# ucl-bug/helmnet

Hardware: AMD Instinct MI355X
Metric: solver iterations/sec (whole node), 256^2 domain batch=32 (higher is better)
Workload: dtype f32

## Files before the change

### helmnet_amd/_lib.py

```python
from __future__ import annotations

import ctypes
import os
from ctypes import POINTER, c_char_p, c_double, c_float, c_int, c_int64, c_size_t, c_void_p

import torch

_LIB_PATH = os.environ.get("HELMNET_HIP_LIB") or os.path.join(os.path.dirname(os.path.abspath(__file__)), "libhelmnet_hip.so")
_lib = None

HN_ACT = {"prelu": 0, "relu": 1, "leakyrelu": 2, "celu": 3, "tanh": 4, "gelu": 5, "tanhshrink": 6, "softplus": 7}
HN_PRECISION = {"fp32": 0, "bf16x3": 1, "fp16": 2, "bf16x2": 3, "valu": 4}
HN_OPTION = {"lanes": 0, "side_stream": 1, "deep": 3, "spectral_pfa": 4, "spectral_radix16": 5, "dc_valu": 6, "spectral_cols": 7, "train_fused": 10, "train_overlap": 11, "dc_pair": 12, "side_sync": 13, "state_kernel": 14, "hist_copy": 15, "inc_sigma_map": 16, "spectral_mixed": 17,
             "graph": 100, "train_lanes": 101, "spectral_plain": 102}
HN_COUNTER = {"graph_replays": 0, "eager_iterations": 1, "graphs_captured": 2, "stream_probes": 3, "side_candidate": 4, "train_fwd_events": 5, "flag_sync_iterations": 6, "spectral_route": 7}
ABI_VERSION = 7
HN_VJP = {"continue": 1, "defer": 2}

SYMBOLS = {
    "hn_abi_version": (c_int, []),
    "hn_create": (c_int, [POINTER(c_void_p), c_int]),
    "hn_destroy": (None, [c_void_p]),
    "hn_last_error": (c_char_p, [c_void_p]),
    "hn_set_unet_precision": (c_int, [c_void_p, c_int]),
    "hn_get_unet_precision": (c_int, [c_void_p]),
    "hn_set_option": (c_int, [c_void_p, c_int, c_int]),
    "hn_get_counter": (c_int64, [c_void_p, c_int]),
    "hn_check_async_errors": (c_int, [c_void_p]),
    "hn_weight_count": (c_size_t, [c_int, c_int, c_int]),
    "hn_load_weights": (c_int, [c_void_p, POINTER(c_float), c_size_t, c_int, c_int, c_int, c_int]),
    "hn_set_domain": (c_int, [c_void_p, c_int, c_int, c_float, c_float]),
    "hn_get_sigmas": (c_int, [c_void_p, c_void_p, c_void_p]),
    "hn_state_len": (c_int64, [c_void_p]),
    "hn_reserve": (c_int, [c_void_p, c_int]),
    "hn_laplacian": (c_int, [c_void_p, c_void_p, c_void_p, c_int, c_void_p]),
    "hn_residual": (c_int, [c_void_p, c_void_p, c_void_p, c_void_p, c_int, c_void_p, c_int, c_void_p]),
    "hn_residual_vjp": (c_int, [c_void_p, c_void_p, c_void_p, c_void_p, c_int, c_void_p]),
    "hn_rmse": (c_int, [c_void_p, c_void_p, c_void_p, c_int, c_void_p]),
    "hn_laplacian_f64": (c_int, [c_void_p, c_void_p, c_void_p, c_int, c_void_p]),
    "hn_residual_f64": (c_int, [c_void_p, c_void_p, c_void_p, c_void_p, c_int, c_void_p, c_void_p, c_int, c_void_p]),
    "hn_gmres_cycle": (c_int, [c_void_p, c_void_p, c_void_p, c_void_p, c_int, c_int, c_int, c_float, c_void_p, c_void_p, c_void_p, c_void_p, c_void_p]),
    "hn_gmres_refine_cycle": (c_int, [c_void_p, c_void_p, c_void_p, c_void_p, c_int, c_int, c_int, c_double, c_float, c_void_p, c_void_p, c_void_p, c_void_p,
                                      c_void_p, c_void_p]),
    "hn_fgmres_cycle": (c_int, [c_void_p, c_void_p, c_void_p, c_void_p, c_int, c_int, c_int, c_float, c_int, c_float, c_void_p, c_void_p, c_void_p, c_void_p,
                                c_void_p, c_void_p]),
    "hn_fgmres_refine_cycle": (c_int, [c_void_p, c_void_p, c_void_p, c_void_p, c_int, c_int, c_int, c_double, c_float, c_int, c_float, c_void_p, c_void_p,
# ... 71 lines not shown
```

### helmnet_amd/csrc/hn_api.hip

```cpp
#include <cmath>
#include <cstdlib>
#include <cstring>

#include <cstdio>
#include "hn_internal.h"

namespace hn {

static thread_local std::string g_err;

void set_global_error(const char* msg) { g_err = msg; }

int fail(hn_ctx* ctx, int code, const char* fmt, ...) {
    char buf[512];
    va_list ap;
    va_start(ap, fmt);
    vsnprintf(buf, sizeof(buf), fmt, ap);
    va_end(ap);
    if (ctx) ctx->err = buf;
    g_err = buf;
    return code;
}

ProfScope::ProfScope(hn_ctx* ctx, int id, hipStream_t st) : c(ctx), s(st) {
// ... 208 lines not shown
    if (!out) return fail(nullptr, HN_ERR_ARG, "hn_create: out is NULL");
    *out = nullptr;
    int count = 0;
    hipError_t e = hipGetDeviceCount(&count);
    if (e != hipSuccess || count == 0)
        return fail(nullptr, HN_ERR_HIP, "hn_create: no HIP device available (%s)", hipGetErrorString(e));
    if (device_id < 0 || device_id >= count) return fail(nullptr, HN_ERR_ARG, "hn_create: device %d of %d", device_id, count);
    hipDeviceProp_t prop;
    if ((e = hipGetDeviceProperties(&prop, device_id)) != hipSuccess)
        return fail(nullptr, HN_ERR_HIP, "hipGetDeviceProperties: %s", hipGetErrorString(e));
    if (std::strncmp(prop.gcnArchName, "gfx950", 6) != 0)
        return fail(nullptr, HN_ERR_UNSUPPORTED, "device %d is %s; this library is built for gfx950 only", device_id, prop.gcnArchName);
    int prev = -1;
    (void)hipGetDevice(&prev);
    if ((e = hipSetDevice(device_id)) != hipSuccess) return fail(nullptr, HN_ERR_HIP, "hipSetDevice: %s", hipGetErrorString(e));
    if (prev >= 0 && prev != device_id) (void)hipSetDevice(prev);
    hn_ctx* c = new (std::nothrow) hn_ctx();
    if (!c) return fail(nullptr, HN_ERR_NOMEM, "out of host memory");
    c->device = device_id;
    *out = c;
    auto bad_env = [&](const char* name, const char* v) {
        const std::string why = c->err;
        hn_destroy(c);
        *out = nullptr;
        return fail(nullptr, HN_ERR_ARG, "hn_create: environment variable %s=%s rejected (%s)", name, v, why.c_str());
    };
    if (const char* v = getenv("HN_UNET_IMPL")) {
        const int mode = std::strcmp(v, "fp32") == 0 ? HN_PREC_FP32 : std::strcmp(v, "bf16x3") == 0 ? HN_PREC_BF16X3 : std::strcmp(v, "fp16") == 0 ? HN_PREC_FP16
                       : std::strcmp(v, "bf16x2") == 0 ? HN_PREC_BF16X2 : std::strcmp(v, "valu") == 0 ? HN_PREC_FP32_VALU : -1;
        if (hn_set_unet_precision(c, mode) != HN_OK) return bad_env("HN_UNET_IMPL", v);
    }
    const struct { const char* env; int opt; } knobs[] = {{"HN_STREAMS", HN_OPT_LANES}, {"HN_SIDE_STREAM", HN_OPT_SIDE_STREAM},
                                                            {"HN_GRAPH", HN_EXP_GRAPH}, {"HN_DEEP", HN_OPT_DEEP},
                                                            {"HN_TRAIN_LANES", HN_EXP_TRAIN_LANES}, {"HN_TRAIN_FUSED", HN_OPT_TRAIN_FUSED}, {"HN_TRAIN_OVERLAP", HN_OPT_TRAIN_OVERLAP}, {"HN_DC_VALU", HN_OPT_DC_VALU}, {"HN_DC_PAIR", HN_OPT_DC_PAIR}, {"HN_SIDE_SYNC", HN_OPT_SIDE_SYNC}, {"HN_STATE_KERNEL", HN_OPT_STATE_KERNEL}, {"HN_HIST_COPY", HN_OPT_HIST_COPY}, {"HN_INC_SIGMA_MAP", HN_OPT_INC_SIGMA_MAP}, {"HN_SPECTRAL_MIXED", HN_OPT_SPECTRAL_MIXED}, {"HN_SPECTRAL_PLAIN", HN_EXP_SPECTRAL_PLAIN}};
    for (const char* name : {"ROCPROF_COUNTER_COLLECTION", "ROCPROF_COUNTERS", "ROCP_METRICS"})
        if (const char* v = getenv(name))
            if (v[0] != '\0' && std::strcmp(v, "0") != 0 && std::strcmp(v, "False") != 0 && std::strcmp(v, "false") != 0) c->opt_side_sync = 0;
    if (const char* v = getenv("HN_SIDE_PRIORITY")) { const int p = std::atoi(v); c->opt_side_priority = p < 0 || p > 3 ? 0 : p; }
    if (const char* v = getenv("HN_DEFER_JOIN")) c->opt_defer_join = std::atoi(v) != 0;
    for (const auto& k : knobs)
        if (const char* v = getenv(k.env)) {
            char* end = nullptr;
            const long n = std::strtol(v, &end, 10);
            if (end == v || *end != '\0') { c->err = "not an integer"; return bad_env(k.env, v); }
            if (hn_set_option(c, k.opt, (int)n) != HN_OK) return bad_env(k.env, v);
        }
    *out = c;
    return HN_OK;
}

int hn_set_unet_precision(hn_ctx* ctx, int precision) {
    if (!ctx) return HN_ERR_ARG;
    if (precision < HN_PREC_FP32 || precision > HN_PREC_FP32_VALU)
        return fail(ctx, HN_ERR_ARG, "hn_set_unet_precision: unknown mode %d", precision);
    if (precision != ctx->precision) clear_step_graphs(ctx);
    ctx->precision = precision;
    return HN_OK;
}

int hn_get_unet_precision(const hn_ctx* ctx) { return ctx ? ctx->precision : HN_ERR_ARG; }

int hn_set_option(hn_ctx* ctx, int option, int value) {
    if (!ctx) return HN_ERR_ARG;
    switch (option) {
        case HN_OPT_LANES:
            if (value < 1 || value > 8) return fail(ctx, HN_ERR_ARG, "HN_OPT_LANES must be in [1, 8] (got %d)", value);
            ctx->opt_lanes = value;
            break;
        case HN_OPT_SIDE_STREAM:
            if (value < 0 || value > 3) return fail(ctx, HN_ERR_ARG, "HN_OPT_SIDE_STREAM must be in [0, 3] (got %d)", value);
            ctx->opt_side_stream = value;
            break;
        case HN_EXP_GRAPH:
            if (value < 0 || value > 64 || (value > 1 && (value & 1)))
                return fail(ctx, HN_ERR_ARG, "HN_EXP_GRAPH must be 0, 1 or an even number of iterations per graph <= 64 (got %d)", value);
            ctx->opt_graph = value;
            break;
        case HN_OPT_DEEP:
            if (value < 0 || value > 2) return fail(ctx, HN_ERR_ARG, "HN_OPT_DEEP must be 0, 1 or 2 (got %d)", value);
            ctx->opt_deep = value;
            break;
        case HN_OPT_SPECTRAL_PFA:
            if (value < 0 || value > 1) return fail(ctx, HN_ERR_ARG, "HN_OPT_SPECTRAL_PFA must be 0 or 1 (got %d)", value);
            ctx->opt_pfa = value;
            break;
        case HN_OPT_SPECTRAL_MIXED:
            if (value < 0 || value > 1) return fail(ctx, HN_ERR_ARG, "HN_OPT_SPECTRAL_MIXED must be 0 or 1 (got %d)", value);
            ctx->opt_mixed = value;
            break;
        case HN_OPT_DC_VALU:
            if (value < 0 || value > 4) return fail(ctx, HN_ERR_ARG, "HN_OPT_DC_VALU must be 0 .. 4 (got %d)", value);
            ctx->opt_dc_valu = value;
            break;
        case HN_OPT_DC_PAIR:
            if (value < 0 || value > 1) return fail(ctx, HN_ERR_ARG, "HN_OPT_DC_PAIR must be 0 or 1 (got %d)", value);
            ctx->opt_dc_pair = value;
            break;
        case HN_OPT_STATE_KERNEL:
            if (value < 0 || value > 1) return fail(ctx, HN_ERR_ARG, "HN_OPT_STATE_KERNEL must be 0 or 1 (got %d)", value);
            ctx->opt_state_kernel = value;
            break;
        case HN_OPT_INC_SIGMA_MAP:
            if (value < 0 || value > 1) return fail(ctx, HN_ERR_ARG, "HN_OPT_INC_SIGMA_MAP must be 0 or 1 (got %d)", value);
            ctx->opt_inc_sigma_map = value;
            break;
        case HN_OPT_HIST_COPY:
            if (value < 0 || value > 1) return fail(ctx, HN_ERR_ARG, "HN_OPT_HIST_COPY must be 0 or 1 (got %d)", value);
            ctx->opt_hist_copy = value;
            break;
        case HN_OPT_SIDE_SYNC:
            if (value < 0 || value > 1) return fail(ctx, HN_ERR_ARG, "HN_OPT_SIDE_SYNC must be 0 or 1 (got %d)", value);
            ctx->opt_side_sync = value;
            break;
        case HN_OPT_SPECTRAL_RADIX16:
            if (value < 0 || value > 2) return fail(ctx, HN_ERR_ARG, "HN_OPT_SPECTRAL_RADIX16 must be 0, 1 or 2 (got %d)", value);
            ctx->opt_radix16 = value;
            break;
        case HN_OPT_SPECTRAL_COLS:
            if (value < 0 || value > 3) return fail(ctx, HN_ERR_ARG, "HN_OPT_SPECTRAL_COLS must be 0, 1, 2 or 3 (got %d)", value);
            ctx->opt_cols_t = value;
            break;
        case HN_EXP_SPECTRAL_PLAIN:
            if (value < 0 || value > 1) return fail(ctx, HN_ERR_ARG, "HN_EXP_SPECTRAL_PLAIN must be 0 or 1 (got %d)", value);
            ctx->opt_spec_plain = value;
            break;
        case HN_EXP_TRAIN_LANES:
            if (value < 1 || value > 2) return fail(ctx, HN_ERR_ARG, "HN_EXP_TRAIN_LANES must be 1 or 2 (got %d)", value);
            ctx->opt_train_lanes = value;
            break;
        case HN_OPT_TRAIN_FUSED:
            if (value < 0 || value > 63) return fail(ctx, HN_ERR_ARG, "HN_OPT_TRAIN_FUSED must be 0 .. 63 (got %d)", value);
            ctx->opt_train_fused = value;
            break;
// ... 730 lines not shown
```

### helmnet_amd/csrc/hn_internal.h

```cpp
#pragma once
#include <hip/hip_runtime.h>

#include <complex>
#include <cstdarg>
#include <cstdint>
#include <cstdio>
#include <string>
#include <vector>

#include "helmnet_hip.h"

namespace hn {

constexpr int kFeat = 8;
constexpr int kCounterStride = 32;
constexpr int kState = 2;
constexpr int kInCh = 6;
constexpr int kMaxDepth = 6;

struct Src {
    const float* p;
    long sb;
    long sc;
    float scale;
// ... 173 lines not shown
    hn::F64Unet* f64 = nullptr;
    hn::KrylovWs* kry = nullptr;
    hn::RefineWs* rfn = nullptr;
    hn::PrecondWs* pcw = nullptr;
    hn::DcLayer inc{}, sig[hn::kMaxDepth]{}, st[hn::kMaxDepth]{}, dec[hn::kMaxDepth + 1]{};
    hn::K8Layer down[hn::kMaxDepth]{}, up[hn::kMaxDepth]{};
    float* fragdev = nullptr;
    const float *f_dec0c = nullptr, *dec0c_b = nullptr;
    const float* v_dec0c = nullptr;
    bool deep_attr_set = false, pfa_attr_set = false, pfa_adj_attr_set = false;
    int precision = HN_PREC_FP32;
    int opt_lanes = 1;
    int opt_side_stream = 1;
    int opt_side_priority = 0;
    int opt_defer_join = 0;
    int opt_graph = 0;
    int opt_pfa = 1;
    int opt_mixed = 0;
    int opt_radix16 = 1;
    int opt_cols_t = 1;
    bool cols_t_attr_set = false, cols512_attr_set = false;
    int opt_spec_plain = 0;
    int opt_deep = 2;
    unsigned* dx_flags = nullptr;
    unsigned* dx_done = nullptr;
    bool deepx_attr_set = false;
    int opt_dc_valu = 4;
    int opt_dc_pair = 1;
    unsigned* pair_flags = nullptr;
    long pair_flags_cap = 0;
    unsigned pair_epoch = 0;
    unsigned* pair_done = nullptr;
    int opt_hist_copy = 0;
    int opt_state_kernel = 1;
    int opt_side_sync = 1;
    unsigned* sync_flags = nullptr;
    unsigned sync_epoch = 0;
    int* sync_err = nullptr;
    int* sync_err_dev = nullptr;
    hn_stream_verdict_rec* stream_tab = nullptr;
    hn_stream_verdict_rec* stream_tab_dev = nullptr;
    int stream_tab_cap = 0;
    float2* inc_sigma_map = nullptr;
    int inc_sigma_band = 0;
    float inc_w_sigma[144]{};
    int opt_inc_sigma_map = 1;
    const float* zero_page = nullptr;
    const float* outc_w = nullptr;
    const float* outc_b = nullptr;
    hn::SpecTables tab;
    int64_t state_len = 0;
    int64_t state_off[hn::kMaxDepth]{};
    int cap_batch = 0;
    float* buf_a[hn::kMaxDepth + 1]{};
    float* buf_o[hn::kMaxDepth]{};
    float* buf_y[hn::kMaxDepth + 1]{};
    float* st_tmp = nullptr;
    struct SideLane {
        hipStream_t stream = nullptr; hipEvent_t ev[hn::kMaxDepth]{}; hipEvent_t done = nullptr;
        bool pending = false;
    };
    SideLane side[8];
    struct SidePick {
        hipStream_t cand[4]{};
        struct Known { hipStream_t ref[3]{}; int nref = 0; int chosen = 0; };
        std::vector<Known> known;
// ... 262 lines not shown
```

### helmnet_amd/csrc/hn_mfma.hip

```cpp
#include <cstdlib>

#include "hn_internal.h"
#include <cstring>
#include <cstdint>

namespace hn {
namespace {

typedef float f32x4 __attribute__((ext_vector_type(4)));
typedef float f32x2 __attribute__((ext_vector_type(2)));

constexpr int cdiv_(int a, int b) { return (a + b - 1) / b; }
constexpr int cmax_(int a, int b) { return a > b ? a : b; }

__device__ __forceinline__ f32x4 mfma4(float a, float b, f32x4 c) {
    return __builtin_amdgcn_mfma_f32_16x16x4f32(a, b, c, 0, 0, 0);
}
__device__ __forceinline__ float div1000(float x) {
    const float r = 1e-3f;
    const float qv = x * r;
    const float e = fmaf(-qv, 1000.0f, x);
    return fmaf(e, r, qv);
}
template <int N>
__device__ __forceinline__ void interleave_mfma_dsread() {
#pragma unroll
    for (int i = 0; i < N; ++i) {
        __builtin_amdgcn_sched_group_barrier(0x008, 1, 0);
        __builtin_amdgcn_sched_group_barrier(0x100, 1, 0);
    }
}

template <int CA, int CB, int CC, int TW>
struct McCfg {
    static constexpr int TH = 16;
    static constexpr int CIN = CA + CB + CC;
    static constexpr int CK = 2;
    static constexpr int NG = cdiv_(CIN, CK);
    static constexpr int IR = TH + 4, PI = TW + 4;
// ... 1636 lines not shown
        for (int gi = 0; gi < C::GW2; ++gi) acc2[gi] = (f32x4){0.f, 0.f, 0.f, 0.f};
        mfma_pairs<C::GW2>(acc2, lds, boff2, MID, MPLANE, PM, F_A2 + 24 * 64, kFeat / 2, lane);
        mfma_pairs<C::GW2>(acc2, lds, boff2, MID + kFeat * MPLANE, MPLANE, PM, F_A2S, kState / 2, lane);
        store(a.dst[1], 2 * q, acc2);
    }
    {
        f32x4 acc2[C::GW2];
#pragma unroll
        for (int gi = 0; gi < C::GW2; ++gi) acc2[gi] = (f32x4){0.f, 0.f, 0.f, 0.f};
        mfma_pairs<C::GW2>(acc2, lds, boff2, MID + kFeat * MPLANE, MPLANE, PM, F_A2S + 6 * 64, kState / 2, lane, 6);
        if (q == 0) store(x.dst, 0, acc2);
    }
}

template <int WX>
struct DnCfg {
    static constexpr int WY = 4 / WX;
    static constexpr int TH = 16, TW = 16 * WX;
    static constexpr int R = TH / WY;
    static constexpr int NWIN = R + 2;
    static constexpr int IR = 2 * TH + 6;
    static constexpr int IC = 2 * TW + 6;
    static constexpr int PI = IC | 1;
    static constexpr int PLANE = IR * PI;
    static constexpr int PLANE_P = PLANE + 64;
    static constexpr int NT = 256;
    static constexpr int NL = cdiv_(IR * IC, NT);
};

template <int WX, bool ALL>
__global__ __launch_bounds__(256, 2) void k_down_mfma(Src in, Dst out, const float* __restrict__ afr ,
                                                       const float* __restrict__ bias, int Hin, int Win, SyncHook hook) {
    using C = DnCfg<WX>;
    sync_hook_begin(hook);
    __shared__ float lds[(ALL ? kFeat : 2) * C::PLANE_P];
    const int tid = threadIdx.x, lane = tid & 63;
    const int wave = __builtin_amdgcn_readfirstlane(tid >> 6);
    const int n = lane & 15, q = lane >> 4;
    const int wx = wave % WX, wy = wave / WX;
    const TileId tl = xcd_tile();
    const int b = tl.z;
    const int X0 = tl.x * C::TW, Y0 = tl.y * C::TH;
    const int Hout = Hin / 2, Wout = Win / 2;

    unsigned gofb[C::NL];
    int lofw[C::NL];
#pragma unroll
    for (int i = 0; i < C::NL; ++i) {
        const int e = tid + i * C::NT;
        const int ir = e / C::IC, ic = e - ir * C::IC;
        const int y = 2 * Y0 - 3 + ir, x = 2 * X0 - 3 + ic;
        const bool inr = e < C::IR * C::IC;
        const bool ok = inr && y >= 0 && y < Hin && x >= 0 && x < Win;
        gofb[i] = ok ? 4u * (unsigned)(y * Win + x) : 0u;
        lofw[i] = ok ? ir * C::PI + ic : C::PLANE + lane;
        if (inr && !ok) {
#pragma unroll
            for (int pl = 0; pl < (ALL ? kFeat : 2); ++pl) lds[pl * C::PLANE_P + ir * C::PI + ic] = 0.f;
        }
    }
    const float* const base = in.p + (long)b * in.sb;
    float stage[C::NL], afrag_next[8];
    auto fetch = [&](int ci) {
        unsigned off[C::NL], aoff = 4u * lane;
#pragma unroll
        for (int i = 0; i < C::NL; ++i) {
            off[i] = gofb[i];
// ... 21 lines not shown
        for (int kx = 0; kx < 8; ++kx) afrag_next[kx] = afr[kx * 64 + lane];
#pragma unroll
        for (int c = 0; c < kFeat; ++c)
#pragma unroll
            for (int i = 0; i < C::NL; ++i) lds[c * C::PLANE_P + lofw[i]] = st[c][i];
        __syncthreads();
    } else {
        fetch(0);
    }
#pragma unroll
    for (int ci = 0; ci < kFeat; ++ci) {
        float* t = lds + (ALL ? ci : (ci & 1)) * C::PLANE_P;
#ifndef HN_DN_ABL
#define HN_DN_ABL 0
#endif
        if (!ALL && !((HN_DN_ABL & 2) && ci >= 2)) {
#pragma unroll
            for (int i = 0; i < C::NL; ++i) t[lofw[i]] = stage[i];
        }
        float afrag[8];
#pragma unroll
        for (int kx = 0; kx < 8; ++kx) afrag[kx] = afrag_next[kx];
        if (!ALL) {
            if (!((HN_DN_ABL & 4) && ci >= 2)) __syncthreads();
            if (ci + 1 < kFeat && !((HN_DN_ABL & 1) && ci >= 1)) fetch(ci + 1);
        } else if (ci + 1 < kFeat) {
#pragma unroll
            for (int kx = 0; kx < 8; ++kx) afrag_next[kx] = afr[((ci + 1) * 8 + kx) * 64 + lane];
        }
        float bv[2][C::NWIN];
#pragma unroll
        for (int wr = 0; wr < C::NWIN; ++wr) bv[0][wr] = t[bbase + 2 * wr * C::PI];
        __builtin_amdgcn_sched_barrier(0);
#pragma unroll
        for (int kx = 0; kx < 8; ++kx) {
            if (kx + 1 < 8) {
#pragma unroll
                for (int wr = 0; wr < C::NWIN; ++wr) bv[(kx + 1) & 1][wr] = t[bbase + 2 * wr * C::PI + kx + 1];
            }
#pragma unroll
            for (int wr = 0; wr < C::NWIN; ++wr) acc[wr] = mfma4(afrag[kx], bv[kx & 1][wr], acc[wr]);
            interleave_mfma_dsread<C::NWIN>();
            __builtin_amdgcn_sched_barrier(0);
        }
    }
    const int X = X0 + 16 * wx + n;
    const float b0 = bias[2 * q], b1 = bias[2 * q + 1];
    if (X < Wout) {
#pragma unroll
        for (int r = 0; r < C::R; ++r) {
            const int Y = Y0 + wy * C::R + r;
            if (Y < Hout) {
                float* p = out.p + (long)b * out.sb + (long)(2 * q) * out.sc + (long)Y * Wout + X;
                p[0] = acc[r][0] + acc[r + 2][1] + b0;
                p[out.sc] = acc[r][2] + acc[r + 2][3] + b1;
            }
        }
    }
}

template <int WX, int R_>
struct UpCfg2 {
    static constexpr int WY = 4 / WX;
    static constexpr int R = R_;
    static constexpr int TH = R * WY, TW = 16 * WX;
    static constexpr int IR = TH + 3;
    static constexpr int IC = TW + 4;
    static constexpr int PI = ((IC + 15) / 32) * 32 + 16;
    static constexpr int PLANE = IR * PI;
    static constexpr int PLANE_P = PLANE + 64;
    static constexpr int NT = 256;
    static constexpr int NL = cdiv_(IR * IC, NT);
};

template <int WX, int R_, bool ALL, bool ACC = false>
__global__ __launch_bounds__(256, 3) void k_up_mfma(Src in, Dst out, const float* __restrict__ afr ,
                                                  const float* __restrict__ bias, int Hin, int Win, SyncHook hook) {
    using C = UpCfg2<WX, R_>;
    __shared__ float lds[(ALL ? kFeat : 4) * C::PLANE_P];
    sync_hook_begin(hook);
    const int tid = threadIdx.x, lane = tid & 63;
    const int wave = __builtin_amdgcn_readfirstlane(tid >> 6);
    const int n = lane & 15, q = lane >> 4;
    const int wx = wave % WX, wy = wave / WX;
    const TileId tl = xcd_tile();
    const int b = tl.z;
    const int X0 = tl.x * C::TW, Yb = tl.y * C::TH - 1;
    const int Hout = 2 * Hin, Wout = 2 * Win;

    unsigned gofb[C::NL];
    int lofw[C::NL];
#pragma unroll
    for (int i = 0; i < C::NL; ++i) {
        const int e = tid + i * C::NT;
        const int ir = e / C::IC, ic = e - ir * C::IC;
        const int y = Yb - 1 + ir, x = X0 - 2 + ic;
        const bool inr = e < C::IR * C::IC;
        const bool ok = inr && y >= 0 && y < Hin && x >= 0 && x < Win;
        gofb[i] = ok ? 4u * (unsigned)(y * Win + x) : 0u;
        lofw[i] = ok ? ir * C::PI + ic : C::PLANE + lane;
        if (inr && !ok) {
#pragma unroll
            for (int pl = 0; pl < (ALL ? kFeat : 4); ++pl) lds[pl * C::PLANE_P + ir * C::PI + ic] = 0.f;
        }
    }
    const float* const base = in.p + (long)b * in.sb;
    float stage[C::NL][2], afrag_next[16];
    auto fetch = [&](int g) {
        unsigned off[C::NL], aoff = 4u * lane;
#pragma unroll
        for (int i = 0; i < C::NL; ++i) {
            off[i] = gofb[i];
            asm volatile("" : "+v"(off[i]));
// ... 24 lines not shown
        for (int j = 0; j < 16; ++j) afrag_next[j] = afr[j * 64 + lane];
#pragma unroll
        for (int c = 0; c < kFeat; ++c)
#pragma unroll
            for (int i = 0; i < C::NL; ++i) lds[c * C::PLANE_P + lofw[i]] = st[c][i];
        __syncthreads();
    } else {
        fetch(0);
    }
#pragma unroll
    for (int g = 0; g < kFeat / 2; ++g) {
        float* t = lds + (ALL ? 2 * g : (g & 1) * 2) * C::PLANE_P;
        if (!ALL) {
#pragma unroll
            for (int i = 0; i < C::NL; ++i) {
                t[lofw[i]] = stage[i][0];
                t[C::PLANE_P + lofw[i]] = stage[i][1];
            }
        }
        float afrag[16];
#pragma unroll
        for (int j = 0; j < 16; ++j) afrag[j] = afrag_next[j];
        if (!ALL) {
            __syncthreads();
            if (g + 1 < kFeat / 2) fetch(g + 1);
        } else if (g + 1 < kFeat / 2) {
#pragma unroll
            for (int j = 0; j < 16; ++j) afrag_next[j] = afr[((g + 1) * 16 + j) * 64 + lane];
        }
        float bv[2][C::R];
#pragma unroll
        for (int wr = 0; wr < C::R; ++wr) bv[0][wr] = t[bbase + wr * C::PI];
        __builtin_amdgcn_sched_barrier(0);
#pragma unroll
        for (int st = 0; st < 10; ++st) {
            const int c = st / 5, o = st % 5;
            if (st + 1 < 10) {
                const int c1 = (st + 1) / 5, o1 = (st + 1) % 5;
#pragma unroll
                for (int wr = 0; wr < C::R; ++wr) bv[(st + 1) & 1][wr] = t[c1 * C::PLANE_P + bbase + wr * C::PI + o1];
            }
#pragma unroll
            for (int wr = 0; wr < C::R; ++wr) {
                if (o < 4) acc[wr][0] = mfma4(afrag[c * 8 + o], bv[st & 1][wr], acc[wr][0]);
                if (o > 0) acc[wr][1] = mfma4(afrag[c * 8 + 4 + (o - 1)], bv[st & 1][wr], acc[wr][1]);
            }
            interleave_mfma_dsread<C::R>();
            __builtin_amdgcn_sched_barrier(0);
        }
    }
    const int X = X0 + 16 * wx + n;
    const float b0 = bias[2 * q], b1 = bias[2 * q + 1];
    if (X < Win) {
#pragma unroll
        for (int wr = 0; wr < C::R; ++wr) {
            const int Y = Yb + wy * C::R + wr;
#pragma unroll
            for (int py = 0; py < 2; ++py) {
                const int y = 2 * Y + 1 + py;
                if (y >= 0 && y < Hout) {
                    float* p = out.p + (long)b * out.sb + (long)(2 * q) * out.sc + (long)y * Wout + 2 * X;
                    float2 o0 = make_float2(acc[wr][0][py] + b0, acc[wr][1][py] + b0);
                    float2 o1 = make_float2(acc[wr][0][2 + py] + b1, acc[wr][1][2 + py] + b1);
                    if (ACC) {
                        const float2 c0 = *reinterpret_cast<const float2*>(p), c1 = *reinterpret_cast<const float2*>(p + out.sc);
                        o0.x += c0.x; o0.y += c0.y; o1.x += c1.x; o1.y += c1.y;
                    }
                    *reinterpret_cast<float2*>(p) = o0;
                    *reinterpret_cast<float2*>(p + out.sc) = o1;
                }
            }
        }
    }
    sync_hook_end(hook);
}

template <typename M>
struct DnX {
    static constexpr int TH = 16, TW = 16, R = 4, NWIN = R + 2;
    static constexpr int IR = 2 * TH + 6, IC = 2 * TW + 6;
    static constexpr int PI = IC | 1;
    static constexpr int ROWB = PI * 16, PARTB = IR * ROWB;
    static constexpr int NL = cdiv_(IR * IC, 256);
    static constexpr int LDS_BYTES = M::NP * PARTB;
};

template <typename M>
__global__ __launch_bounds__(256, 2) void k_down_x16(Src in, Dst out, const void* __restrict__ afr ,
                                                      const float* __restrict__ bias, int Hin, int Win) {
    using C = DnX<M>;
    typedef typename M::V8 V8;
    typedef typename M::T T;
    __shared__ __attribute__((aligned(16))) unsigned char lds[C::LDS_BYTES];
    const int tid = threadIdx.x, lane = tid & 63;
    const int wy = __builtin_amdgcn_readfirstlane(tid >> 6);
    const int n = lane & 15, q = lane >> 4;
    const TileId tl = xcd_tile();
    const int b = tl.z;
    const int X0 = tl.x * C::TW, Y0 = tl.y * C::TH;
    const int Hout = Hin / 2, Wout = Win / 2;
    const float* const base = in.p + (long)b * in.sb;
    float v[C::NL][kFeat];
#pragma unroll
    for (int i = 0; i < C::NL; ++i) {
        const int e = tid + i * 256;
        const int ir = e / C::IC, ic = e - ir * C::IC;
// ... 410 lines not shown
    else launch_dc8_bwd_n<2>(a, H, W, batch, s);
    HN_HIP(ctx, hipGetLastError());
    return HN_OK;
}

int launch_dc8_bwd_aux(hn_ctx* ctx, const McBwd& a, const McBwdAux& x, int H, int W, int batch, hipStream_t s) {
    if (!dc8_bwd_applies(H, W) || a.dst[0].nch != kFeat || a.dst[1].nch != kFeat || x.dst.nch != kState)
        return fail(ctx, HN_ERR_ARG, "internal: the decoder + hidden-state backward kernel needs channel groups 8 | 8 and 2");
    int tw, tx, ty;
    dc8_bwd_shape(H, W, tw, tx, ty);
    const int nt = tx * ty * batch;
    const bool gen = a.act > HN_ACT_LEAKYRELU;
    if (tw == 32) {
        if (gen) hipLaunchKernelGGL((k_dc_bwd_mfma_aux<8, 32, true>), dim3(nt), dim3(256), 0, s, a, x, H, W, tx, ty, nt);
        else hipLaunchKernelGGL((k_dc_bwd_mfma_aux<8, 32, false>), dim3(nt), dim3(256), 0, s, a, x, H, W, tx, ty, nt);
    } else {
        if (gen) hipLaunchKernelGGL((k_dc_bwd_mfma_aux<8, 16, true>), dim3(nt), dim3(256), 0, s, a, x, H, W, tx, ty, nt);
        else hipLaunchKernelGGL((k_dc_bwd_mfma_aux<8, 16, false>), dim3(nt), dim3(256), 0, s, a, x, H, W, tx, ty, nt);
    }
    HN_HIP(ctx, hipGetLastError());
    return HN_OK;
}

void launch_down(const hn_ctx* ctx, Src in, Dst out, const K8Frag& w, int Hin, int Win, int batch, hipStream_t s, SyncHook hook) {
    const int Wout = Win / 2, Hout = Hin / 2;
    const float *frag = w.f32, *bias = w.bias;
    const int mode = w.f16 != nullptr ? ctx->precision : HN_PREC_FP32;
    if ((mode == HN_PREC_FP16 || mode == HN_PREC_BF16X2) && Wout >= 64) {
        const dim3 g(cdiv_(Wout, 16), cdiv_(Hout, 16), batch);
        if (mode == 3) hipLaunchKernelGGL((k_down_x16<SplitBf16x2>), g, dim3(256), 0, s, in, out, w.bf16, bias, Hin, Win);
        else hipLaunchKernelGGL((k_down_x16<HalfF16>), g, dim3(256), 0, s, in, out, w.f16, bias, Hin, Win);
        return;
    }
    if (Wout > 64) hipLaunchKernelGGL((k_down_mfma<4, false>), dim3(cdiv_(Wout, 64), cdiv_(Hout, 16), batch), dim3(256), 0, s, in, out, frag, bias, Hin, Win, hook);
    else if (Wout > 32) {
        const dim3 g(cdiv_(Wout, 32), cdiv_(Hout, 16), batch);
        hipLaunchKernelGGL((k_down_mfma<2, false>), g, dim3(256), 0, s, in, out, frag, bias, Hin, Win, hook);
    }
    else {
        const dim3 g(cdiv_(Wout, 16), cdiv_(Hout, 16), batch);
        hipLaunchKernelGGL((k_down_mfma<1, true>), g, dim3(256), 0, s, in, out, frag, bias, Hin, Win, hook);
    }
}

void launch_up(const hn_ctx* ctx, Src in, Dst out, const K8Frag& w, int Hin, int Win, int batch, hipStream_t s, bool accumulate, SyncHook hook) {
    const float *frag = w.f32, *bias = w.bias;
    const int mode = w.f16 != nullptr ? ctx->precision : HN_PREC_FP32;
    if (mode >= HN_PREC_BF16X3 && mode <= HN_PREC_BF16X2 && Win >= 64) {
        const dim3 g(cdiv_(Win, 16), cdiv_(Hin + 1, 20), batch);
        if (mode == 1) hipLaunchKernelGGL((k_up_x16<SplitBf16>), g, dim3(256), 0, s, in, out, w.bf16, bias, Hin, Win, hook);
        else if (mode == 3) hipLaunchKernelGGL((k_up_x16<SplitBf16x2>), g, dim3(256), 0, s, in, out, w.bf16, bias, Hin, Win, hook);
        else hipLaunchKernelGGL((k_up_x16<HalfF16>), g, dim3(256), 0, s, in, out, w.f16, bias, Hin, Win, hook);
        return;
    }
    constexpr int up_small = 64;
    if (Win > up_small) {
        const dim3 g(cdiv_(Win, 32), cdiv_(Hin + 1, 22), batch);
        if (accumulate) hipLaunchKernelGGL((k_up_mfma<2, 11, false, true>), g, dim3(256), 0, s, in, out, frag, bias, Hin, Win, hook);
        else hipLaunchKernelGGL((k_up_mfma<2, 11, false>), g, dim3(256), 0, s, in, out, frag, bias, Hin, Win, hook);
    } else {
        const dim3 g(cdiv_(Win, 16), cdiv_(Hin + 1, 20), batch);
        if (accumulate) hipLaunchKernelGGL((k_up_mfma<1, 5, true, true>), g, dim3(256), 0, s, in, out, frag, bias, Hin, Win, hook);
        else hipLaunchKernelGGL((k_up_mfma<1, 5, true>), g, dim3(256), 0, s, in, out, frag, bias, Hin, Win, hook);
    }
}

}
```

### include/helmnet_hip.h

```cpp
#ifndef HELMNET_HIP_H
#define HELMNET_HIP_H

#include <stddef.h>
#include <stdint.h>

#ifdef __cplusplus
extern "C" {
#endif

typedef struct hn_ctx hn_ctx;

enum hn_status {
    HN_OK = 0,
    HN_ERR_ARG = -1,
    HN_ERR_STATE = -2,
    HN_ERR_UNSUPPORTED = -3,
    HN_ERR_HIP = -4,
    HN_ERR_NOMEM = -5
};

enum hn_act { HN_ACT_PRELU = 0, HN_ACT_RELU = 1, HN_ACT_LEAKYRELU = 2, HN_ACT_CELU = 3, HN_ACT_TANH = 4, HN_ACT_GELU = 5,
              HN_ACT_TANHSHRINK = 6, HN_ACT_SOFTPLUS = 7 };

enum hn_precision { HN_PREC_FP32 = 0, HN_PREC_BF16X3 = 1, HN_PREC_FP16 = 2, HN_PREC_BF16X2 = 3, HN_PREC_FP32_VALU = 4 };

enum hn_option {
    HN_OPT_LANES = 0,
    HN_OPT_SIDE_STREAM = 1,
    HN_OPT_DEEP = 3,
    HN_OPT_SPECTRAL_PFA = 4,
    HN_OPT_SPECTRAL_MIXED = 17,
    HN_OPT_SPECTRAL_RADIX16 = 5,
    HN_OPT_DC_VALU = 6,
    HN_OPT_DC_PAIR = 12,
    HN_OPT_SIDE_SYNC = 13,
    HN_OPT_STATE_KERNEL = 14,
    HN_OPT_HIST_COPY = 15,
    HN_OPT_INC_SIGMA_MAP = 16,
    HN_OPT_SPECTRAL_COLS = 7,
    HN_OPT_TRAIN_FUSED = 10,
    HN_OPT_TRAIN_OVERLAP = 11,
    HN_EXP_GRAPH = 100,
    HN_EXP_TRAIN_LANES = 101,
    HN_EXP_SPECTRAL_PLAIN = 102
};
enum hn_counter { HN_CNT_GRAPH_REPLAYS = 0, HN_CNT_EAGER_ITERATIONS = 1, HN_CNT_GRAPHS_CAPTURED = 2,
                  HN_CNT_STREAM_PROBES = 3,
                  HN_CNT_SIDE_CANDIDATE = 4,
                  HN_CNT_TRAIN_FWD_EVENTS = 5,
                  HN_CNT_FLAG_SYNC_ITERATIONS = 6,
                  HN_CNT_SPECTRAL_ROUTE = 7 };

#define HN_ABI_VERSION 7
int hn_abi_version(void);

int hn_create(hn_ctx** out, int device_id);
void hn_destroy(hn_ctx* ctx);
const char* hn_last_error(const hn_ctx* ctx);

size_t hn_weight_count(int features, int depth, int state_ch);

int hn_load_weights(hn_ctx* ctx, const float* blob, size_t n_floats, int features, int depth,
                    int state_ch, int act_kind);

int hn_set_unet_precision(hn_ctx* ctx, int precision);
int hn_get_unet_precision(const hn_ctx* ctx);
int hn_set_option(hn_ctx* ctx, int option, int value);
int64_t hn_get_counter(const hn_ctx* ctx, int counter);
int hn_check_async_errors(hn_ctx* ctx);

int hn_set_domain(hn_ctx* ctx, int n, int pml, float sigma_max, float k);
// ... 96 lines not shown
```

Baseline: 2235.

## Add split-window 8x8 down conv and row-grouped up conv kernels behind conv8 option

Adds k_down_split, a strided 8x8 down-convolution whose output tile is split across wavefronts by window rows, with a hand-over of partial sums through LDS. It also adds k_up_rows, a transposed-conv kernel that stages all feature planes into LDS once, keeps all A-fragments in registers and processes rows in groups of four. Both are enabled by default through a new conv8 option, with the old kernels kept as fallbacks. The intent is better occupancy and more data reuse in the UNet conv stages, at the cost of more registers and LDS per block and an extra LDS hand-over step. Compile-gated timing trace macros are also added.

```diff
diff --git a/helmnet_amd/_lib.py b/helmnet_amd/_lib.py
--- a/helmnet_amd/_lib.py
+++ b/helmnet_amd/_lib.py
@@ -11,7 +11,7 @@
 
 HN_ACT = {"prelu": 0, "relu": 1, "leakyrelu": 2, "celu": 3, "tanh": 4, "gelu": 5, "tanhshrink": 6, "softplus": 7}
 HN_PRECISION = {"fp32": 0, "bf16x3": 1, "fp16": 2, "bf16x2": 3, "valu": 4}
-HN_OPTION = {"lanes": 0, "side_stream": 1, "deep": 3, "spectral_pfa": 4, "spectral_radix16": 5, "dc_valu": 6, "spectral_cols": 7, "train_fused": 10, "train_overlap": 11, "dc_pair": 12, "side_sync": 13, "state_kernel": 14, "hist_copy": 15, "inc_sigma_map": 16, "spectral_mixed": 17,
+HN_OPTION = {"lanes": 0, "side_stream": 1, "deep": 3, "spectral_pfa": 4, "spectral_radix16": 5, "dc_valu": 6, "spectral_cols": 7, "train_fused": 10, "train_overlap": 11, "dc_pair": 12, "side_sync": 13, "state_kernel": 14, "hist_copy": 15, "inc_sigma_map": 16, "spectral_mixed": 17, "conv8": 18,
              "graph": 100, "train_lanes": 101, "spectral_plain": 102}
 HN_COUNTER = {"graph_replays": 0, "eager_iterations": 1, "graphs_captured": 2, "stream_probes": 3, "side_candidate": 4, "train_fwd_events": 5, "flag_sync_iterations": 6, "spectral_route": 7}
 ABI_VERSION = 7
diff --git a/helmnet_amd/csrc/hn_api.hip b/helmnet_amd/csrc/hn_api.hip
--- a/helmnet_amd/csrc/hn_api.hip
+++ b/helmnet_amd/csrc/hn_api.hip
@@ -264,7 +264,7 @@
     }
     const struct { const char* env; int opt; } knobs[] = {{"HN_STREAMS", HN_OPT_LANES}, {"HN_SIDE_STREAM", HN_OPT_SIDE_STREAM},
                                                             {"HN_GRAPH", HN_EXP_GRAPH}, {"HN_DEEP", HN_OPT_DEEP},
-                                                            {"HN_TRAIN_LANES", HN_EXP_TRAIN_LANES}, {"HN_TRAIN_FUSED", HN_OPT_TRAIN_FUSED}, {"HN_TRAIN_OVERLAP", HN_OPT_TRAIN_OVERLAP}, {"HN_DC_VALU", HN_OPT_DC_VALU}, {"HN_DC_PAIR", HN_OPT_DC_PAIR}, {"HN_SIDE_SYNC", HN_OPT_SIDE_SYNC}, {"HN_STATE_KERNEL", HN_OPT_STATE_KERNEL}, {"HN_HIST_COPY", HN_OPT_HIST_COPY}, {"HN_INC_SIGMA_MAP", HN_OPT_INC_SIGMA_MAP}, {"HN_SPECTRAL_MIXED", HN_OPT_SPECTRAL_MIXED}, {"HN_SPECTRAL_PLAIN", HN_EXP_SPECTRAL_PLAIN}};
+                                                            {"HN_TRAIN_LANES", HN_EXP_TRAIN_LANES}, {"HN_TRAIN_FUSED", HN_OPT_TRAIN_FUSED}, {"HN_TRAIN_OVERLAP", HN_OPT_TRAIN_OVERLAP}, {"HN_DC_VALU", HN_OPT_DC_VALU}, {"HN_DC_PAIR", HN_OPT_DC_PAIR}, {"HN_SIDE_SYNC", HN_OPT_SIDE_SYNC}, {"HN_STATE_KERNEL", HN_OPT_STATE_KERNEL}, {"HN_HIST_COPY", HN_OPT_HIST_COPY}, {"HN_INC_SIGMA_MAP", HN_OPT_INC_SIGMA_MAP}, {"HN_SPECTRAL_MIXED", HN_OPT_SPECTRAL_MIXED}, {"HN_CONV8", HN_OPT_CONV8}, {"HN_SPECTRAL_PLAIN", HN_EXP_SPECTRAL_PLAIN}};
     for (const char* name : {"ROCPROF_COUNTER_COLLECTION", "ROCPROF_COUNTERS", "ROCP_METRICS"})
         if (const char* v = getenv(name))
             if (v[0] != '\0' && std::strcmp(v, "0") != 0 && std::strcmp(v, "False") != 0 && std::strcmp(v, "false") != 0) c->opt_side_sync = 0;
@@ -331,6 +331,10 @@
         case HN_OPT_STATE_KERNEL:
             if (value < 0 || value > 1) return fail(ctx, HN_ERR_ARG, "HN_OPT_STATE_KERNEL must be 0 or 1 (got %d)", value);
             ctx->opt_state_kernel = value;
+            break;
+        case HN_OPT_CONV8:
+            if (value < 0 || value > 1) return fail(ctx, HN_ERR_ARG, "HN_OPT_CONV8 must be 0 or 1 (got %d)", value);
+            ctx->opt_conv8 = value;
             break;
         case HN_OPT_INC_SIGMA_MAP:
             if (value < 0 || value > 1) return fail(ctx, HN_ERR_ARG, "HN_OPT_INC_SIGMA_MAP must be 0 or 1 (got %d)", value);
diff --git a/helmnet_amd/csrc/hn_internal.h b/helmnet_amd/csrc/hn_internal.h
--- a/helmnet_amd/csrc/hn_internal.h
+++ b/helmnet_amd/csrc/hn_internal.h
@@ -229,6 +229,7 @@
     unsigned pair_epoch = 0;
     unsigned* pair_done = nullptr;
     int opt_hist_copy = 0;
+    int opt_conv8 = 1;
     int opt_state_kernel = 1;
     int opt_side_sync = 1;
     unsigned* sync_flags = nullptr;
diff --git a/helmnet_amd/csrc/hn_mfma.hip b/helmnet_amd/csrc/hn_mfma.hip
--- a/helmnet_amd/csrc/hn_mfma.hip
+++ b/helmnet_amd/csrc/hn_mfma.hip
@@ -5,6 +5,14 @@
 #include <cstdint>
 
 namespace hn {
+#ifdef HN_C8TRACE
+__device__ unsigned long long g_c8_trace[4][2048][5];
+#define C8_T(i) do { if (threadIdx.x == 0) g_c8_trace[C8_SLOT][(blockIdx.x + gridDim.x * (blockIdx.y + gridDim.y * blockIdx.z)) & 2047][i] = __builtin_amdgcn_s_memrealtime(); } while (0)
+#define C8_END() do { __builtin_amdgcn_s_waitcnt(0); C8_T(4); } while (0)
+#else
+#define C8_T(i) do { } while (0)
+#define C8_END() do { } while (0)
+#endif
 namespace {
 
 typedef float f32x4 __attribute__((ext_vector_type(4)));
@@ -1707,7 +1715,9 @@
 __global__ __launch_bounds__(256, 2) void k_down_mfma(Src in, Dst out, const float* __restrict__ afr ,
                                                        const float* __restrict__ bias, int Hin, int Win, SyncHook hook) {
     using C = DnCfg<WX>;
+    constexpr int C8_SLOT = WX == 4 ? 0 : 1; (void)C8_SLOT;
     sync_hook_begin(hook);
+    C8_T(0);
     __shared__ float lds[(ALL ? kFeat : 2) * C::PLANE_P];
     const int tid = threadIdx.x, lane = tid & 63;
     const int wave = __builtin_amdgcn_readfirstlane(tid >> 6);
@@ -1795,6 +1805,7 @@
 #pragma unroll
         for (int wr = 0; wr < C::NWIN; ++wr) bv[0][wr] = t[bbase + 2 * wr * C::PI];
         __builtin_amdgcn_sched_barrier(0);
+        if (ci == 0) C8_T(1);
 #pragma unroll
         for (int kx = 0; kx < 8; ++kx) {
             if (kx + 1 < 8) {
@@ -1807,6 +1818,7 @@
             __builtin_amdgcn_sched_barrier(0);
         }
     }
+    C8_T(2);
     const int X = X0 + 16 * wx + n;
     const float b0 = bias[2 * q], b1 = bias[2 * q + 1];
     if (X < Wout) {
@@ -1820,6 +1832,8 @@
             }
         }
     }
+    C8_T(3);
+    C8_END();
 }
 
 template <int WX, int R_>
@@ -1840,8 +1854,10 @@
 __global__ __launch_bounds__(256, 3) void k_up_mfma(Src in, Dst out, const float* __restrict__ afr ,
                                                   const float* __restrict__ bias, int Hin, int Win, SyncHook hook) {
     using C = UpCfg2<WX, R_>;
+    constexpr int C8_SLOT = WX == 2 ? 2 : 3; (void)C8_SLOT;
     __shared__ float lds[(ALL ? kFeat : 4) * C::PLANE_P];
     sync_hook_begin(hook);
+    C8_T(0);
     const int tid = threadIdx.x, lane = tid & 63;
     const int wave = __builtin_amdgcn_readfirstlane(tid >> 6);
     const int n = lane & 15, q = lane >> 4;
@@ -1932,6 +1948,7 @@
 #pragma unroll
         for (int wr = 0; wr < C::R; ++wr) bv[0][wr] = t[bbase + wr * C::PI];
         __builtin_amdgcn_sched_barrier(0);
+        if (g == 0) C8_T(1);
 #pragma unroll
         for (int st = 0; st < 10; ++st) {
             const int c = st / 5, o = st % 5;
@@ -1949,6 +1966,7 @@
             __builtin_amdgcn_sched_barrier(0);
         }
     }
+    C8_T(2);
     const int X = X0 + 16 * wx + n;
     const float b0 = bias[2 * q], b1 = bias[2 * q + 1];
     if (X < Win) {
@@ -1972,6 +1990,246 @@
             }
         }
     }
+    C8_T(3);
+    C8_END();
+    sync_hook_end(hook);
+}
+
+template <int WX, int TH_>
+struct DnCfgS {
+    static constexpr int WY = 4 / WX;
+    static constexpr int TH = TH_, TW = 16 * WX;
+    static constexpr int S = (TH + 2) / WY;
+    static_assert(S * WY == TH + 2 && S >= 2 && WY >= 2, "the window rows split evenly and a hand-over reaches one wavefront down");
+    static constexpr int IR = 2 * TH + 6;
+    static constexpr int IC = 2 * TW + 6;
+    static constexpr int PI = IC | 1;
+    static constexpr int PLANE = IR * PI;
+    static constexpr int PLANE_P = PLANE + 64;
+    static constexpr int NT = 256;
+    static constexpr int NL = cdiv_(IR * IC, NT);
+    static_assert(2 * PLANE_P >= 4 * 4 * 64, "the hand-over (4 wavefronts x 4 values per lane) fits the staging buffers");
+};
+
+template <int WX, int TH_, int MINB>
+__global__ __launch_bounds__(256, MINB) void k_down_split(Src in, Dst out, const float* __restrict__ afr ,
+                                                           const float* __restrict__ bias, int Hin, int Win, SyncHook hook) {
+    using C = DnCfgS<WX, TH_>;
+    constexpr int C8_SLOT = TH_ == 16 ? 0 : 1; (void)C8_SLOT;
+    sync_hook_begin(hook);
+    C8_T(0);
+    __shared__ float lds[2 * C::PLANE_P];
+    const int tid = threadIdx.x, lane = tid & 63;
+    const int wave = __builtin_amdgcn_readfirstlane(tid >> 6);
+    const int n = lane & 15, q = lane >> 4;
+    const int wx = wave % WX, wy = wave / WX;
+    const TileId tl = xcd_tile();
+    const int b = tl.z;
+    const int X0 = tl.x * C::TW, Y0 = tl.y * C::TH;
+    const int Hout = Hin / 2, Wout = Win / 2;
+
+    unsigned gofb[C::NL];
+    int lofw[C::NL];
+#pragma unroll
+    for (int i = 0; i < C::NL; ++i) {
+        const int e = tid + i * C::NT;
+        const int ir = e / C::IC, ic = e - ir * C::IC;
+        const int y = 2 * Y0 - 3 + ir, x = 2 * X0 - 3 + ic;
+        const bool inr = e < C::IR * C::IC;
+        const bool ok = inr && y >= 0 && y < Hin && x >= 0 && x < Win;
+        gofb[i] = ok ? 4u * (unsigned)(y * Win + x) : 0u;
+        lofw[i] = ok ? ir * C::PI + ic : C::PLANE + lane;
+        if (inr && !ok) lds[ir * C::PI + ic] = lds[C::PLANE_P + ir * C::PI + ic] = 0.f;
+    }
+    const float* const base = in.p + (long)b * in.sb;
+    float stage[C::NL], afrag_next[8];
+    auto fetch = [&](int ci) {
+        unsigned off[C::NL], aoff = 4u * lane;
+#pragma unroll
+        for (int i = 0; i < C::NL; ++i) {
+            off[i] = gofb[i];
+            asm volatile("" : "+v"(off[i]));
+        }
+        asm volatile("" : "+v"(aoff));
+        const char* p0 = reinterpret_cast<const char*>(base + (long)ci * in.sc);
+#pragma unroll
+        for (int i = 0; i < C::NL; ++i) stage[i] = *reinterpret_cast<const float*>(p0 + off[i]);
+#pragma unroll
+        for (int kx = 0; kx < 8; ++kx) afrag_next[kx] = *reinterpret_cast<const float*>(reinterpret_cast<const char*>(afr + (ci * 8 + kx) * 64) + aoff);
+    };
+    const int bbase = (2 * wy * C::S + q) * C::PI + 2 * (16 * wx + n);
+    f32x4 acc[C::S];
+#pragma unroll
+    for (int i = 0; i < C::S; ++i) acc[i] = (f32x4){0.f, 0.f, 0.f, 0.f};
+
+    fetch(0);
+#pragma unroll
+    for (int ci = 0; ci < kFeat; ++ci) {
+        float* t = lds + (ci & 1) * C::PLANE_P;
+#pragma unroll
+        for (int i = 0; i < C::NL; ++i) t[lofw[i]] = stage[i];
+        float afrag[8];
+#pragma unroll
+        for (int kx = 0; kx < 8; ++kx) afrag[kx] = afrag_next[kx];
+        __syncthreads();
+        if (ci + 1 < kFeat) fetch(ci + 1);
+        float bv[2][C::S];
+#pragma unroll
+        for (int wr = 0; wr < C::S; ++wr) bv[0][wr] = t[bbase + 2 * wr * C::PI];
+        __builtin_amdgcn_sched_barrier(0);
+        if (ci == 0) C8_T(1);
+#pragma unroll
+        for (int kx = 0; kx < 8; ++kx) {
+            if (kx + 1 < 8) {
+#pragma unroll
+                for (int wr = 0; wr < C::S; ++wr) bv[(kx + 1) & 1][wr] = t[bbase + 2 * wr * C::PI + kx + 1];
+            }
+#pragma unroll
+            for (int wr = 0; wr < C::S; ++wr) acc[wr] = mfma4(afrag[kx], bv[kx & 1][wr], acc[wr]);
+            interleave_mfma_dsread<C::S>();
+            __builtin_amdgcn_sched_barrier(0);
+        }
+    }
+    C8_T(2);
+    __syncthreads();
+    if (wy > 0) {
+#pragma unroll
+        for (int j = 0; j < 2; ++j) {
+            lds[((wave * 2 + j) * 2 + 0) * 64 + lane] = acc[j][1];
+            lds[((wave * 2 + j) * 2 + 1) * 64 + lane] = acc[j][3];
+        }
+    }
+    __syncthreads();
+    const int X = X0 + 16 * wx + n;
+    const float b0 = bias[2 * q], b1 = bias[2 * q + 1];
+    if (X < Wout) {
+#pragma unroll
+        for (int i = 0; i < C::S; ++i) {
+            const int r = wy * C::S + i, Y = Y0 + r;
+            if (r < C::TH && Y < Hout) {
+                float p10, p11;
+                if (i + 2 < C::S) { p10 = acc[i + 2][1]; p11 = acc[i + 2][3]; }
+                else {
+                    const int j = i + 2 - C::S;
+                    p10 = lds[(((wave + WX) * 2 + j) * 2 + 0) * 64 + lane];
+                    p11 = lds[(((wave + WX) * 2 + j) * 2 + 1) * 64 + lane];
+                }
+                float* p = out.p + (long)b * out.sb + (long)(2 * q) * out.sc + (long)Y * Wout + X;
+                p[0] = acc[i][0] + p10 + b0;
+                p[out.sc] = acc[i][2] + p11 + b1;
+            }
+        }
+    }
+    C8_T(3);
+    C8_END();
+}
+
+template <int WX, int R_, int RG, bool ACC = false>
+__global__ __launch_bounds__(256, 3) void k_up_rows(Src in, Dst out, const float* __restrict__ afr ,
+                                                     const float* __restrict__ bias, int Hin, int Win, SyncHook hook) {
+    using C = UpCfg2<WX, R_>;
+    constexpr int C8_SLOT = WX == 2 ? 2 : 3; (void)C8_SLOT;
+    __shared__ float lds[kFeat * C::PLANE_P];
+    sync_hook_begin(hook);
+    C8_T(0);
+    const int tid = threadIdx.x, lane = tid & 63;
+    const int wave = __builtin_amdgcn_readfirstlane(tid >> 6);
+    const int n = lane & 15, q = lane >> 4;
+    const int wx = wave % WX, wy = wave / WX;
+    const TileId tl = xcd_tile();
+    const int b = tl.z;
+    const int X0 = tl.x * C::TW, Yb = tl.y * C::TH - 1;
+    const int Hout = 2 * Hin, Wout = 2 * Win;
+    const float* const base = in.p + (long)b * in.sb;
+    {
+        float st[kFeat][C::NL];
+        int lofw[C::NL];
+#pragma unroll
+        for (int i = 0; i < C::NL; ++i) {
+            const int e = tid + i * C::NT;
+            const int ir = e / C::IC, ic = e - ir * C::IC;
+            const int y = Yb - 1 + ir, x = X0 - 2 + ic;
+            const bool inr = e < C::IR * C::IC;
+            const bool ok = inr && y >= 0 && y < Hin && x >= 0 && x < Win;
+            const unsigned gofb = ok ? 4u * (unsigned)(y * Win + x) : 0u;
+            lofw[i] = ok ? ir * C::PI + ic : C::PLANE + lane;
+#pragma unroll
+            for (int c = 0; c < kFeat; ++c) st[c][i] = *reinterpret_cast<const float*>(reinterpret_cast<const char*>(base + (long)c * in.sc) + gofb);
+            if (inr && !ok) {
+#pragma unroll
+                for (int pl = 0; pl < kFeat; ++pl) lds[pl * C::PLANE_P + ir * C::PI + ic] = 0.f;
+            }
+        }
+#pragma unroll
+        for (int c = 0; c < kFeat; ++c)
+#pragma unroll
+            for (int i = 0; i < C::NL; ++i) lds[c * C::PLANE_P + lofw[i]] = st[c][i];
+    }
+    float afrag[64];
+#pragma unroll
+    for (int j = 0; j < 64; ++j) afrag[j] = afr[j * 64 + lane];
+    const int X = X0 + 16 * wx + n;
+    const float b0 = bias[2 * q], b1 = bias[2 * q + 1];
+    float* const obase = out.p + (long)b * out.sb + (long)(2 * q) * out.sc + 2 * X;
+    __syncthreads();
+    const int bbase = (wy * C::R + q) * C::PI + 16 * wx + n;
+#pragma unroll
+    for (int r0 = 0; r0 < C::R; r0 += RG) {
+        constexpr int NSTEP = (kFeat / 2) * 10;
+        const float* t = lds + bbase + r0 * C::PI;
+        f32x4 acc[RG][2];
+        float bv[2][RG];
+#pragma unroll
+        for (int wr = 0; wr < RG; ++wr) {
+            acc[wr][0] = acc[wr][1] = (f32x4){0.f, 0.f, 0.f, 0.f};
+            if (r0 + wr < C::R) bv[0][wr] = t[wr * C::PI];
+        }
+        __builtin_amdgcn_sched_barrier(0);
+        if (r0 == 0) C8_T(1);
+#pragma unroll
+        for (int s = 0; s < NSTEP; ++s) {
+            const int g = s / 10, c = (s % 10) / 5, o = s % 5;
+            if (s + 1 < NSTEP) {
+                const int pl1 = 2 * ((s + 1) / 10) + ((s + 1) % 10) / 5, o1 = (s + 1) % 5;
+#pragma unroll
+                for (int wr = 0; wr < RG; ++wr)
+                    if (r0 + wr < C::R) bv[(s + 1) & 1][wr] = t[pl1 * C::PLANE_P + wr * C::PI + o1];
+            }
+#pragma unroll
+            for (int wr = 0; wr < RG; ++wr) {
+                if (r0 + wr >= C::R) continue;
+                if (o < 4) acc[wr][0] = mfma4(afrag[g * 16 + c * 8 + o], bv[s & 1][wr], acc[wr][0]);
+                if (o > 0) acc[wr][1] = mfma4(afrag[g * 16 + c * 8 + 4 + (o - 1)], bv[s & 1][wr], acc[wr][1]);
+            }
+            interleave_mfma_dsread<RG>();
+            __builtin_amdgcn_sched_barrier(0);
+        }
+        if (r0 + RG >= C::R) C8_T(2);
+        if (X < Win) {
+#pragma unroll
+            for (int wr = 0; wr < RG; ++wr) {
+                if (r0 + wr >= C::R) continue;
+                const int Y = Yb + wy * C::R + r0 + wr;
+#pragma unroll
+                for (int py = 0; py < 2; ++py) {
+                    const int y = 2 * Y + 1 + py;
+                    if (y >= 0 && y < Hout) {
+                        float* p = obase + (long)y * Wout;
+                        float2 o0 = make_float2(acc[wr][0][py] + b0, acc[wr][1][py] + b0);
+                        float2 o1 = make_float2(acc[wr][0][2 + py] + b1, acc[wr][1][2 + py] + b1);
+                        if (ACC) {
+                            const float2 c0 = *reinterpret_cast<const float2*>(p), c1 = *reinterpret_cast<const float2*>(p + out.sc);
+                            o0.x += c0.x; o0.y += c0.y; o1.x += c1.x; o1.y += c1.y;
+                        }
+                        *reinterpret_cast<float2*>(p) = o0;
+                        *reinterpret_cast<float2*>(p + out.sc) = o1;
+                    }
+                }
+            }
+        }
+    }
+    C8_T(3);
+    C8_END();
     sync_hook_end(hook);
 }
 
@@ -2448,10 +2706,13 @@
         else hipLaunchKernelGGL((k_down_x16<HalfF16>), g, dim3(256), 0, s, in, out, w.f16, bias, Hin, Win);
         return;
     }
-    if (Wout > 64) hipLaunchKernelGGL((k_down_mfma<4, false>), dim3(cdiv_(Wout, 64), cdiv_(Hout, 16), batch), dim3(256), 0, s, in, out, frag, bias, Hin, Win, hook);
+    if (Wout > 64) {
+        if (ctx->opt_conv8) hipLaunchKernelGGL((k_down_split<2, 16, 4>), dim3(cdiv_(Wout, 32), cdiv_(Hout, 16), batch), dim3(256), 0, s, in, out, frag, bias, Hin, Win, hook);
+        else hipLaunchKernelGGL((k_down_mfma<4, false>), dim3(cdiv_(Wout, 64), cdiv_(Hout, 16), batch), dim3(256), 0, s, in, out, frag, bias, Hin, Win, hook);
+    }
     else if (Wout > 32) {
-        const dim3 g(cdiv_(Wout, 32), cdiv_(Hout, 16), batch);
-        hipLaunchKernelGGL((k_down_mfma<2, false>), g, dim3(256), 0, s, in, out, frag, bias, Hin, Win, hook);
+        if (ctx->opt_conv8) hipLaunchKernelGGL((k_down_split<2, 8, 4>), dim3(cdiv_(Wout, 32), cdiv_(Hout, 8), batch), dim3(256), 0, s, in, out, frag, bias, Hin, Win, hook);
+        else hipLaunchKernelGGL((k_down_mfma<2, false>), dim3(cdiv_(Wout, 32), cdiv_(Hout, 16), batch), dim3(256), 0, s, in, out, frag, bias, Hin, Win, hook);
     }
     else {
         const dim3 g(cdiv_(Wout, 16), cdiv_(Hout, 16), batch);
@@ -2472,7 +2733,11 @@
     constexpr int up_small = 64;
     if (Win > up_small) {
         const dim3 g(cdiv_(Win, 32), cdiv_(Hin + 1, 22), batch);
-        if (accumulate) hipLaunchKernelGGL((k_up_mfma<2, 11, false, true>), g, dim3(256), 0, s, in, out, frag, bias, Hin, Win, hook);
+        if (ctx->opt_conv8) {
+            if (accumulate) hipLaunchKernelGGL((k_up_rows<2, 11, 4, true>), g, dim3(256), 0, s, in, out, frag, bias, Hin, Win, hook);
+            else hipLaunchKernelGGL((k_up_rows<2, 11, 4>), g, dim3(256), 0, s, in, out, frag, bias, Hin, Win, hook);
+        }
+        else if (accumulate) hipLaunchKernelGGL((k_up_mfma<2, 11, false, true>), g, dim3(256), 0, s, in, out, frag, bias, Hin, Win, hook);
         else hipLaunchKernelGGL((k_up_mfma<2, 11, false>), g, dim3(256), 0, s, in, out, frag, bias, Hin, Win, hook);
     } else {
         const dim3 g(cdiv_(Win, 16), cdiv_(Hin + 1, 20), batch);
@@ -2482,3 +2747,9 @@
 }
 
 }
+
+#ifdef HN_C8TRACE
+extern "C" int hn_debug_c8_trace(unsigned long long* dst) {
+    return (int)hipMemcpyFromSymbol(dst, HIP_SYMBOL(hn::g_c8_trace), sizeof(unsigned long long) * 4 * 2048 * 5);
+}
+#endif
diff --git a/include/helmnet_hip.h b/include/helmnet_hip.h
--- a/include/helmnet_hip.h
+++ b/include/helmnet_hip.h
@@ -37,6 +37,7 @@
     HN_OPT_STATE_KERNEL = 14,
     HN_OPT_HIST_COPY = 15,
     HN_OPT_INC_SIGMA_MAP = 16,
+    HN_OPT_CONV8 = 18,
     HN_OPT_SPECTRAL_COLS = 7,
     HN_OPT_TRAIN_FUSED = 10,
     HN_OPT_TRAIN_OVERLAP = 11,
```

Measured after the change: 2230. About the same (-0.2%).
